# rajan-dubey8/camouflage-multimodal

Measured on AMD Instinct MI355X. Metric: images/sec fwd+bwd (fusion model train step: fwd + loss + bwd + clip + AdamW), higher is better.
Workload: dtype bf16; 1 GPU; BASELINE configs[1] on the path that exists (SURVEY 8d): cross-attention fusion model, packed variable-Nr minibatch (Nr ~ real 303..530 histogram, mean 483), Nk=13 real KG rows, train mode dropout 0.3, random-init weights; batch_per_gpu=16, global_batch=16, rg_dim=128, hidden_dim=256, num_heads=8, parallelism=dp1, precision=bf16 MFMA operands, fp32 accumulate/optimizer

## Files before the change

camouflage_multimodal_amd/csrc/common.h:

```cpp
#pragma once
#include <hip/hip_runtime.h>
#include <stdint.h>

#define CAMO_WAVE 64

enum : uint32_t {
  SITE_ATTN_RG2KG = 1, SITE_ATTN_KG2RG = 2, SITE_FFN_RG = 3, SITE_FFN_KG = 4, SITE_FUSE = 5,
  SITE_HEAD0 = 6,
  SITE_LATE0 = 10
};
enum : uint32_t { SITE_RGT_CONV0 = 32 , SITE_RGT_SHARED = 36, SITE_RGT_HEADS = 37 };

struct DropCfg {
  uint32_t seed_lo, seed_hi;
  float p;
  float scale;
  uint32_t thr;
};

__host__ __device__ inline DropCfg make_drop(int training, float p, uint64_t seed) {
  DropCfg d;
  d.seed_lo = (uint32_t)(seed & 0xFFFFFFFFull);
  d.seed_hi = (uint32_t)(seed >> 32);
  d.p = (training && p > 0.f) ? p : 0.f;
  d.scale = d.p > 0.f ? 1.0f / (1.0f - d.p) : 1.0f;
  const double t = (double)d.p * 16777216.0;
  unsigned long long t24 = (unsigned long long)t;
  if ((double)t24 < t) ++t24;
  d.thr = t24 >= 16777216ull ? 0xFFFFFFFFu : (uint32_t)(t24 << 8);
  return d;
}

__device__ __forceinline__ uint32_t fmix32(uint32_t x) {
  x ^= x >> 16; x *= 0x85EBCA6Bu; x ^= x >> 13; x *= 0xC2B2AE35u; x ^= x >> 16;
  return x;
}

__device__ __forceinline__ float drop_mult(const DropCfg& d, uint32_t site, uint32_t idx) {
  const uint32_t x = fmix32((idx + (site * 0x85EBCA77u + d.seed_lo)) ^ d.seed_hi);
  return x >= d.thr ? d.scale : 0.0f;
}

extern "C" __device__ int camo_writelane_i32(int, int, int) __asm("llvm.amdgcn.writelane.i32");
#define SET_LANE(v, s, i) (v) = (uint32_t)camo_writelane_i32((int)(s), (i), (int)(v))

__device__ __forceinline__ float wave_sum(float v) {
#pragma unroll
  for (int o = 32; o > 0; o >>= 1) v += __shfl_xor(v, o, 64);
  return v;
}
template <int CTRL, int ROWMASK>
__device__ __forceinline__ float dpp_add(float v) {
  return v + __int_as_float(__builtin_amdgcn_update_dpp(0, __float_as_int(v), CTRL, ROWMASK, 0xf, true));
}
__device__ __forceinline__ float wave_sum_lane63(float v) {
  v = dpp_add<0x111, 0xf>(v);
  v = dpp_add<0x112, 0xf>(v);
  v = dpp_add<0x114, 0xf>(v);
  v = dpp_add<0x118, 0xf>(v);
  v = dpp_add<0x142, 0xa>(v);
  v = dpp_add<0x143, 0xc>(v);
  return v;
}
__device__ __forceinline__ float wave_max(float v) {
// ... 65 lines not shown
```

camouflage_multimodal_amd/csrc/fused_rows.hip:

```cpp
#include "fused_rows.h"
#include "shadow_inl.h"
#include "gemm.h"
#include "mfma_inl.h"

namespace {

template <int NT, int KS, bool W_IS_A, int DEPTH, bool USE_ROT = true>
struct Stage {
  static constexpr int TOTAL = NT * KS;
  static constexpr int D = DEPTH < TOTAL ? DEPTH : TOTAL;
  static_assert(!USE_ROT || (KS & (KS - 1)) == 0, "rotated k order: power-of-two k steps");
  u32x4 buf[D];
  const u32x4* wp; int rot;
  __device__ __forceinline__ int keff(int ks) const { return USE_ROT ? ((ks + rot) & (KS - 1)) : ks; }
  __device__ __forceinline__ const u32x4* wptr(int i) const { return wp + 64 * (keff(i / NT) * NT + (i % NT)); }
  __device__ __forceinline__ void prefetch(const u32x4* __restrict__ wp_, int rot_) {
    wp = wp_; rot = rot_;
#pragma unroll
    for (int i = 0; i < D; ++i) buf[i] = *wptr(i);
  }
  __device__ __forceinline__ void run(const char* act, f32x16 (&acc)[NT]) {
    run_f([&](int ks) { return *reinterpret_cast<const bf16x8*>(act + 32 * ks); }, acc);
  }
  template <class F>
  __device__ __forceinline__ void run_f(F&& frag, f32x16 (&acc)[NT]) {
    bf16x8 x = frag(keff(0)), xn = x;
#pragma unroll
    for (int i = 0; i < TOTAL; ++i) {
      const int ks = i / NT, t = i % NT;
      const bf16x8 wf = as_frag(buf[i % D]);
      if (i + D < TOTAL) buf[i % D] = *wptr(i + D);
      if (t == 0) {
        x = xn;
        if (ks + 1 < KS) xn = frag(keff(ks + 1));
      }
      if constexpr (W_IS_A) acc[t] = __builtin_amdgcn_mfma_f32_32x32x16_bf16(wf, x, acc[t], 0, 0, 0);
      else                  acc[t] = __builtin_amdgcn_mfma_f32_32x32x16_bf16(x, wf, acc[t], 0, 0, 0);
      __builtin_amdgcn_sched_barrier(0);
    }
  }
};

__device__ __forceinline__ void stamp(unsigned long long* stamps, int k) {
  if (stamps && threadIdx.x == 0) stamps[(size_t)blockIdx.x * 8 + k] = __builtin_amdgcn_s_memrealtime();
}

template <int LOG2C>
__device__ __forceinline__ void copy_out(const char* lds, int pitch, int col_byte0, us16* dst, int ld, size_t row0, int nrows) {
  for (int c = threadIdx.x; c < (32 << LOG2C); c += 256) {
    const int r = c >> LOG2C, k = c & ((1 << LOG2C) - 1);
    if (r < nrows)
      store16_wt(reinterpret_cast<char*>(dst + (row0 + r) * (size_t)ld) + 16 * k, *reinterpret_cast<const u32x4*>(lds + r * pitch + col_byte0 + 16 * k));
  }
}

__global__ __launch_bounds__(256) void shadow_kernel(const ShadowBatch sb, int total_chunks) {
  const int gid = blockIdx.x * 256 + threadIdx.x;
  for (int zi = 0; zi < sb.nzero; ++zi) {
    u32x4* z = static_cast<u32x4*>(sb.zero_ptr[zi]);
    const size_t n16 = sb.zero_bytes[zi] >> 4;
    for (size_t i = gid; i < n16; i += (size_t)gridDim.x * 256) z[i] = u32x4{0u, 0u, 0u, 0u};
  }
  if (gid >= total_chunks) return;
  int ji = 0;
#pragma unroll
  for (int i = 1; i < SHADOW_MAXJ; ++i)
    if (i < sb.n && gid >= sb.j[i].chunk_begin) ji = i;
// ... 7 lines not shown
  extern __shared__ __attribute__((aligned(16))) char smem[];
  const FrontStream& S = a.s[(int)blockIdx.x >= a.s[1].tile_begin ? 1 : 0];
  const int tid = threadIdx.x, lane = tid & 63, l31 = lane & 31, h = lane >> 5;
  const int w = __builtin_amdgcn_readfirstlane(tid >> 6);
  const int row0 = ((int)blockIdx.x - S.tile_begin) * 32;
  const int nrows = min(32, S.M - row0);
  char* bufX = smem; char* bufR = smem + F_BUFR; char* bufQ = smem + F_BUFQ;
  const int rot = ROT ? (int)(blockIdx.x >> 3) : 0;
  stamp(a.stamps, 0);
  Stage<2, 8, true, DEPTH> st0;
  st0.prefetch(reinterpret_cast<const u32x4*>(S.W0) + (size_t)w * (8 * 2 * 64) + lane, rot);
  float* ptab = reinterpret_cast<float*>(smem + F_PTAB);
  {
    const int r = tid >> 3, c = tid & 7;
    const float4* src = reinterpret_cast<const float4*>(S.X + (size_t)(row0 + min(r, nrows - 1)) * 128 + 16 * c);
    float4 v0 = src[0], v1 = src[1], v2 = src[2], v3 = src[3];
    const float p0 = S.b0[tid], p1 = S.bq[tid], p2 = S.bkv[tid], p3 = S.bkv[256 + tid];
    ptab[tid] = p0; ptab[256 + tid] = p1; ptab[512 + tid] = p2; ptab[768 + tid] = p3;
    if (r >= nrows) { v0 = v1 = v2 = v3 = make_float4(0.f, 0.f, 0.f, 0.f); }
    *reinterpret_cast<u32x4*>(bufX + r * PX + 32 * c) = u32x4{pack2(v0.x, v0.y), pack2(v0.z, v0.w), pack2(v1.x, v1.y), pack2(v1.z, v1.w)};
    *reinterpret_cast<u32x4*>(bufX + r * PX + 32 * c + 16) = u32x4{pack2(v2.x, v2.y), pack2(v2.z, v2.w), pack2(v3.x, v3.y), pack2(v3.z, v3.w)};
  }
  __syncthreads();
  Stage<6, 16, true, DEPTH> st1;
  {
    f32x16 acc[2] = {zero16(), zero16()};
    st0.run(bufX + l31 * PX + 16 * h, acc);
    st1.prefetch(reinterpret_cast<const u32x4*>(S.W1) + (size_t)w * (16 * 6 * 64) + lane, rot);
#pragma unroll
    for (int t = 0; t < 2; ++t)
#pragma unroll
      for (int g = 0; g < 4; ++g) {
        const int c0 = 64 * w + 32 * t + 8 * g + 4 * h;
        const float4 bv = *reinterpret_cast<const float4*>(ptab + c0);
        *reinterpret_cast<u32x2*>(bufR + l31 * PR + 2 * c0) =
            u32x2{pack2(acc[t][4 * g] + bv.x, acc[t][4 * g + 1] + bv.y), pack2(acc[t][4 * g + 2] + bv.z, acc[t][4 * g + 3] + bv.w)};
      }
  }
  __syncthreads();
  stamp(a.stamps, 1);
  {
    f32x16 acc[6];
#pragma unroll
    for (int t = 0; t < 6; ++t) acc[t] = zero16();
    st1.run(bufR + l31 * PR + 16 * h, acc);
#pragma unroll
    for (int t = 0; t < 6; ++t) {
      const int tg = 6 * w + t;
      const float* bias = ptab + 256 + 32 * tg;
      const float sc = tg < 8 ? a.qscale : 1.0f;
#pragma unroll
      for (int g = 0; g < 4; ++g) {
        const int c = 8 * g + 4 * h;
        const float4 bv = *reinterpret_cast<const float4*>(bias + c);
        *reinterpret_cast<u32x2*>(bufQ + l31 * PQ + 2 * (32 * tg + c)) =
            u32x2{pack2((acc[t][4 * g] + bv.x) * sc, (acc[t][4 * g + 1] + bv.y) * sc),
                  pack2((acc[t][4 * g + 2] + bv.z) * sc, (acc[t][4 * g + 3] + bv.w) * sc)};
      }
    }
  }
  __syncthreads();
  stamp(a.stamps, 2);
  copy_out<5>(bufQ, PQ, 0, S.Q16, 256, row0, nrows);
  copy_out<6>(bufQ, PQ, 512, S.KV16, 512, row0, nrows);
  copy_out<5>(bufR, PR, 0, S.R16, 256, row0, nrows);
  if (a.save) copy_out<4>(bufX, PX, 0, S.X16, 128, row0, nrows);
  for (int zi = 0; zi < a.nzero; ++zi) {
    u32x4* z = static_cast<u32x4*>(a.zero_ptr[zi]);
    const unsigned n16 = a.zero_bytes[zi] >> 4;
    for (unsigned i = blockIdx.x * 256 + tid; i < n16; i += gridDim.x * 256) z[i] = u32x4{0u, 0u, 0u, 0u};
  }
  stamp(a.stamps, 3);
}

constexpr int PK = 528;
constexpr int PVC = 192;
constexpr int PT = 260;
constexpr int B_VS = 16 * PK;
template <int OCC> struct BackL;
template <> struct BackL<2> { static constexpr int XH = 0, O = 32 * PT * 4, Y = O + 32 * PR, RED = Y + 32 * PR, PTAB = RED + 1024, LDS = PTAB + 5120; };
template <> struct BackL<3> { static constexpr int Y = 0, XH = 32 * PR, O = 2 * 32 * PR, RED = O + 32 * PR, LDS = RED + 1024; };
constexpr int B_LDS = BackL<2>::LDS;
// ... 62 lines not shown
  const us16* kbase = a.KV2_16 + (size_t)rb * 512 + 64 * w + 8 * h;
  const us16* vbase = a.KV2_16 + (size_t)rb * 512 + 256 + 64 * w;
  bf16x8 qf[2][2];
  u32x4 kf[2][2][2], vv[2][4];
#pragma unroll
  for (int hd = 0; hd < 2; ++hd)
#pragma unroll
    for (int s = 0; s < 2; ++s) qf[hd][s] = as_frag(*reinterpret_cast<const u32x4*>(qrow + 32 * hd + 16 * s));
#pragma unroll
  for (int c = 0; c < 2; ++c) {
    const us16* p = kbase + (size_t)min(r0 + 32 * c + l31, nr - 1) * 512;
#pragma unroll
    for (int hd = 0; hd < 2; ++hd)
#pragma unroll
      for (int s = 0; s < 2; ++s) kf[c][hd][s] = *reinterpret_cast<const u32x4*>(p + 32 * hd + 16 * s);
  }
#pragma unroll
  for (int c = 0; c < 2; ++c)
#pragma unroll
    for (int i = 0; i < 4; ++i) {
      const int id = lane + 64 * i;
      vv[c][i] = *reinterpret_cast<const u32x4*>(vbase + (size_t)min(r0 + 32 * c + (id >> 3), nr - 1) * 512 + 8 * (id & 7));
    }
  f32x16 S[2][2];
  float mx[2] = {-INFINITY, -INFINITY};
#pragma unroll
  for (int c = 0; c < 2; ++c)
#pragma unroll
    for (int hd = 0; hd < 2; ++hd) {
      S[c][hd] = zero16();
#pragma unroll
      for (int s = 0; s < 2; ++s) S[c][hd] = __builtin_amdgcn_mfma_f32_32x32x16_bf16(as_frag(kf[c][hd][s]), qf[hd][s], S[c][hd], 0, 0, 0);
#pragma unroll
      for (int i = 0; i < 16; ++i) mx[hd] = (r0 + 32 * c + acc_row(i, h) < nr) ? fmaxf(mx[hd], S[c][hd][i]) : mx[hd];
    }
  mx[0] = fmaxf(mx[0], __shfl_xor(mx[0], 32, 64));
  mx[1] = fmaxf(mx[1], __shfl_xor(mx[1], 32, 64));
  stamp(a.stamps, 1);
  f32x16 Z[2] = {zero16(), zero16()};
  float L[2] = {0.f, 0.f};
  const bool dodrop = a.drop.p > 0.f;
  const int q4 = (lane >> 2) & 3, p4 = lane & 3, g1 = (lane >> 4) & 1;
#pragma unroll
  for (int c = 0; c < 2; ++c) {
#pragma unroll
    for (int i = 0; i < 4; ++i) { const int id = lane + 64 * i; *reinterpret_cast<u32x4*>(Vt + (id >> 3) * PVC + 16 * (id & 7)) = vv[c][i]; }
#pragma unroll
    for (int hd = 0; hd < 2; ++hd) {
      float e[16];
#pragma unroll
      for (int i = 0; i < 16; ++i) {
        const int row = r0 + 32 * c + acc_row(i, h);
        e[i] = row < nr ? __expf(S[c][hd][i] - mx[hd]) : 0.f;
        L[hd] += e[i];
        if (dodrop) e[i] *= drop_mult(a.drop, SITE_ATTN_KG2RG, ((uint32_t)(rb + row) * 8u + (uint32_t)(2 * w + hd)) * (uint32_t)Nk + (uint32_t)l31);
      }
#pragma unroll
      for (int s = 0; s < 2; ++s) {
        const bf16x8 ef = as_frag(u32x4{pack2(e[8 * s], e[8 * s + 1]), pack2(e[8 * s + 2], e[8 * s + 3]),
                                        pack2(e[8 * s + 4], e[8 * s + 5]), pack2(e[8 * s + 6], e[8 * s + 7])});
        const char* vp = Vt + (16 * s + 4 * h + q4) * PVC + 2 * (32 * hd + 16 * g1 + 4 * p4);
        const bf16x8 vf = join(lds_tr16(vp), lds_tr16(vp + 8 * PVC));
        Z[hd] = __builtin_amdgcn_mfma_f32_32x32x16_bf16(ef, vf, Z[hd], 0, 0, 0);
      }
    }
  }
  L[0] += __shfl_xor(L[0], 32, 64);
  L[1] += __shfl_xor(L[1], 32, 64);
  stamp(a.stamps, 2);
#pragma unroll
  for (int hd = 0; hd < 2; ++hd) {
    float* part = a.part + (((size_t)a.tile_off[b] + 2 * sp) * 8 + 2 * w + hd) * PART_FLOATS;
    if (lane < 16) {
      __hip_atomic_store(part + lane, mx[hd], __ATOMIC_RELAXED, __HIP_MEMORY_SCOPE_AGENT);
      __hip_atomic_store(part + 16 + lane, L[hd], __ATOMIC_RELAXED, __HIP_MEMORY_SCOPE_AGENT);
    }
    float* zt = reinterpret_cast<float*>(Vt);
#pragma unroll
// ... 81 lines not shown
      *reinterpret_cast<u32x2*>(bufO + j * PR + 2 * (32 * hd + 4 * f4)) =
          u32x2{pack2(acc[it][0] * il, acc[it][1] * il), pack2(acc[it][2] * il, acc[it][3] * il)};
    }
  }
}

template <int DEPTH, bool ROT, int OCC>
__global__ __launch_bounds__(256, OCC) void back_kernel(const BackArgs a) {
  extern __shared__ __attribute__((aligned(16))) char smem[];
  const int tid = threadIdx.x, lane = tid & 63, l31 = lane & 31, h = lane >> 5;
  const int w = __builtin_amdgcn_readfirstlane(tid >> 6);
  const int nkg = a.B * a.max_splits;
  const int vid = (int)blockIdx.x < a.lead_tiles ? nkg + (int)blockIdx.x : ((int)blockIdx.x < a.lead_tiles + nkg ? (int)blockIdx.x - a.lead_tiles : (int)blockIdx.x);
  const bool kg = vid < nkg;
  int rot = ROT ? (int)(blockIdx.x >> 3) : 0;
  using L = BackL<OCC>;
  char* bufO = smem + L::O; char* bufY = smem + L::Y;
  float* red = reinterpret_cast<float*>(smem + L::RED);
  float* tile32 = reinterpret_cast<float*>(smem);
  int b; size_t rowg0; int nrows; float inv_n;
  stamp(a.stamps, 0);
  const BackStream& S = a.s[kg ? 1 : 0];
  Stage<2, 16, true, DEPTH> sto;
  Stage<4, 16, false, DEPTH> stf;
  if (!kg) sto.prefetch(reinterpret_cast<const u32x4*>(S.Wo) + (size_t)w * (16 * 2 * 64) + lane, rot);
  float* ptab = reinterpret_cast<float*>(smem + BackL<2>::PTAB);
  float pt[5];
  u32x2 rres[2][4];
  auto load_early = [&](size_t row) {
    if constexpr (OCC == 2) {
      pt[0] = S.bo[tid]; pt[1] = S.ln_g[tid]; pt[2] = S.ln_b[tid]; pt[3] = S.b1[tid]; pt[4] = S.b1[256 + tid];
#pragma unroll
      for (int t = 0; t < 2; ++t)
#pragma unroll
        for (int g = 0; g < 4; ++g) rres[t][g] = *reinterpret_cast<const u32x2*>(S.R16 + row * 256 + 64 * w + 32 * t + 8 * g + 4 * h);
    }
  };
  if (kg) {
    b = vid / a.max_splits;
    const int sp = vid - b * a.max_splits;
    if (ROT) rot = b;
    const int nsplit = (a.off[b + 1] - a.off[b] + SPLIT_ROWS - 1) / SPLIT_ROWS;
    if (sp >= nsplit) return;
    attn_kg_split(a, smem, b, sp, w, lane);
    stamp(a.stamps, 4);
    asm volatile("s_waitcnt vmcnt(0)" ::: "memory");
    __syncthreads();
// ... 17 lines not shown
    const int4 td = a.tile_desc[vid - nkg];
    if (td.x < 0) return;
    b = td.x; rowg0 = td.y; nrows = td.z; inv_n = __int_as_float(td.w);
    load_early(rowg0 + min(l31, nrows - 1));
    attn_rg_tile(a, smem, bufO, b, rowg0, nrows, w, lane);
  }
  if constexpr (OCC == 2) {
#pragma unroll
    for (int i = 0; i < 5; ++i) ptab[256 * i + tid] = pt[i];
  }
  __syncthreads();
  stamp(a.stamps, 1);
  auto pvec = [&](const float* g, int at, int c) {
    if constexpr (OCC == 2) return *reinterpret_cast<const float4*>(ptab + at + c);
    else return *reinterpret_cast<const float4*>(g + c);
  };

  const size_t rrow = rowg0 + min(l31, nrows - 1);
  float u[32];
  float rstd_keep = 0.f;
  {
    f32x16 acc[2] = {zero16(), zero16()};
    sto.run(bufO + l31 * PR + 16 * h, acc);
    stf.prefetch(reinterpret_cast<const u32x4*>(S.W1) + (size_t)w * (16 * 4 * 64) + lane, rot);
    float part = 0.f;
#pragma unroll
    for (int t = 0; t < 2; ++t)
#pragma unroll
      for (int g = 0; g < 4; ++g) {
        const int c0 = 64 * w + 32 * t + 8 * g + 4 * h;
        const float4 bv = pvec(S.bo, 0, c0);
        u32x2 rv;
        if constexpr (OCC == 2) rv = rres[t][g];
        else rv = *reinterpret_cast<const u32x2*>(S.R16 + rrow * 256 + c0);
        float* o = u + 16 * t + 4 * g;
        o[0] = acc[t][4 * g] + bv.x + bf_lo(rv.x); o[1] = acc[t][4 * g + 1] + bv.y + bf_hi(rv.x);
        o[2] = acc[t][4 * g + 2] + bv.z + bf_lo(rv.y); o[3] = acc[t][4 * g + 3] + bv.w + bf_hi(rv.y);
        part += (o[0] + o[1]) + (o[2] + o[3]);
      }
    auto row_total = [&](float p, int slot) {
      p += __shfl_xor(p, 32, 64);
      if (h == 0) red[slot * 128 + w * 32 + l31] = p;
      __syncthreads();
      return (red[slot * 128 + l31] + red[slot * 128 + 32 + l31]) + (red[slot * 128 + 64 + l31] + red[slot * 128 + 96 + l31]);
    };
    const float mean = row_total(part, 0) * (1.0f / 256.0f);
    float sq = 0.f;
// ... 31 lines not shown
          const float send = up ? ys[i] : ys[i + n];
          const float keep = up ? ys[i + n] : ys[i];
          ys[i] = keep + __shfl_xor(send, m, 64);
        }
      }
      const float tot = ys[0] + __shfl_xor(ys[0], 1, 64);
      if ((l31 & 1) == 0) {
        const int i16 = (l31 >> 1) & 15;
        atomicAdd(S.Ymean + (size_t)b * 256 + 64 * w + 32 * t + 8 * (i16 >> 2) + 4 * h + (i16 & 3), tot * inv_n);
      }
    }
  }
  __syncthreads();
  stamp(a.stamps, 2);
  float ymean_keep = 0.f;
  if constexpr (OCC == 2) {
    float sum = 0.f;
    for (int r = 0; r < nrows; ++r) sum += tile32[r * PT + tid];
    ymean_keep = sum * inv_n;
  }

  {
    f32x16 acc[4] = {zero16(), zero16(), zero16(), zero16()};
    stf.run(bufY + l31 * PR + 16 * h, acc);
    if constexpr (OCC == 2) atomicAdd(S.Ymean + (size_t)b * 256 + tid, ymean_keep);
    const bool dodrop = a.drop.p > 0.f;
#pragma unroll
    for (int t = 0; t < 4; ++t) {
      const int f = 128 * w + 32 * t + l31;
      float bias;
      if constexpr (OCC == 2) bias = ptab[768 + f];
      else bias = S.b1[f];
      float colsum = 0.f;
      uint32_t wlo = 0u, whi = 0u;
#pragma unroll
      for (int i = 0; i < 16; ++i) {
        if (8 * (i >> 2) >= nrows) continue;
        const int row = acc_row(i, h);
        float v = fmaxf(acc[t][i] + bias, 0.f);
        if (dodrop) v *= drop_mult(a.drop, S.site_ffn, (uint32_t)(rowg0 + row) * 512u + (uint32_t)f);
        if (row >= nrows) v = 0.f;
        colsum += v;
        if (a.save) {
          const unsigned long long bal = __ballot(v > 0.f);
          SET_LANE(wlo, (uint32_t)bal, i); SET_LANE(whi, (uint32_t)(bal >> 32), i);
        }
      }
      colsum += __shfl_xor(colsum, 32, 64);
      if (h == 0) atomicAdd(S.Hmean + (size_t)b * 512 + f, colsum * inv_n);
      if (a.save && lane < 16) {
        const int ra = acc_row(lane, 0);
        if (ra < nrows) S.mask[(rowg0 + ra) * 16 + 4 * w + t] = wlo;
        if (ra + 4 < nrows) S.mask[(rowg0 + ra + 4) * 16 + 4 * w + t] = whi;
      }
    }
  }
  if (a.save) {
    char* bufXH = smem + L::XH;
    if (w == 0 && h == 0 && l31 < nrows) S.rstd[rowg0 + l31] = rstd_keep;
    __syncthreads();
    if constexpr (OCC == 2) {
#pragma unroll
      for (int t = 0; t < 2; ++t)
#pragma unroll
        for (int g = 0; g < 4; ++g) {
          const float* o = u + 16 * t + 4 * g;
          *reinterpret_cast<u32x2*>(bufXH + l31 * PR + 2 * (64 * w + 32 * t + 8 * g + 4 * h)) = u32x2{pack2(o[0], o[1]), pack2(o[2], o[3])};
        }
      __syncthreads();
    }
    copy_out<5>(bufXH, PR, 0, S.XH16, 256, rowg0, nrows);
    copy_out<5>(bufO, PR, 0, S.O16, 256, rowg0, nrows);
    copy_out<5>(bufY, PR, 0, S.Y16, 256, rowg0, nrows);
  }
  stamp(a.stamps, 3);
}
// ... 117 lines not shown
  const bool rok = l31 < nrows;
  float* ptab = reinterpret_cast<float*>(smem + W_PTAB);
  const float rstd = S.rstd[vrow];
  const float ptv0 = S.dcomb[(size_t)b * S.ld_dcomb + tid], ptv1 = S.ln_g[tid];
  u32x2 xv[2][4], ov[2][4];
#pragma unroll
  for (int t = 0; t < 2; ++t)
#pragma unroll
    for (int g = 0; g < 4; ++g) {
      const int c0 = 64 * w + 32 * t + 8 * g + 4 * h;
      xv[t][g] = *reinterpret_cast<const u32x2*>(S.XH16 + vrow * 256 + c0);
    }
  if (kg) {
#pragma unroll
    for (int t = 0; t < 2; ++t)
#pragma unroll
      for (int g = 0; g < 4; ++g) ov[t][g] = *reinterpret_cast<const u32x2*>(a.O2_16 + vrow * 256 + 64 * w + 32 * t + 8 * g + 4 * h);
  }
  const float dh0 = S.dHm[(size_t)b * S.ld_dHm + tid], dh1 = S.dHm[(size_t)b * S.ld_dHm + 256 + tid];
  u32x4 mw[4];
#pragma unroll
  for (int i = 0; i < 4; ++i) mw[i] = reinterpret_cast<const u32x4*>(S.mask + vrow * 16)[i];
  u32x4 qreg[4];
  if (!kg) {
#pragma unroll
    for (int i = 0; i < 4; ++i) {
      const int id = tid + 256 * i;
      qreg[i] = *reinterpret_cast<const u32x4*>(a.Q16 + (rowg0 + min(id >> 5, nrows - 1)) * 256 + 8 * (id & 31));
    }
    u32x4 kv[4];
#pragma unroll
    for (int i = 0; i < 4; ++i) {
      const int c = tid + 256 * i;
      kv[i] = *reinterpret_cast<const u32x4*>(a.KV16 + ((size_t)b * a.Nk + min(c >> 6, a.Nk - 1)) * 512 + 8 * (c & 63));
    }
#pragma unroll
    for (int i = 0; i < 4; ++i) {
      const int c = tid + 256 * i, j = c >> 6, ch = c & 63;
      const u32x4 v = j < a.Nk ? kv[i] : u32x4{0u, 0u, 0u, 0u};
      if (ch < 32) *reinterpret_cast<u32x4*>(Ks + j * PK + 16 * ch) = v;
      else         *reinterpret_cast<u32x4*>(Vs + j * PK + 16 * (ch - 32)) = v;
    }
  }
  {
    const float gs = inv_n * a.drop.scale;
    gtab[tid] = f2bf(dh0 * gs); gtab[256 + tid] = f2bf(dh1 * gs);
  }
  ptab[tid] = ptv0; ptab[256 + tid] = ptv1;
#pragma unroll
  for (int t = 0; t < 2; ++t)
#pragma unroll
    for (int g = 0; g < 4; ++g) {
      const int c0 = 64 * w + 32 * t + 8 * g + 4 * h;
      *reinterpret_cast<u32x2*>(bufdU + l31 * PR + 2 * c0) = xv[t][g];
      if (kg) *reinterpret_cast<u32x2*>(Ks + l31 * PR + 2 * c0) = ov[t][g];
    }
  __syncthreads();
// ... 86 lines not shown
        dot = fmaf(acc2[t][4 * g], bf_lo(ov.x), dot); dot = fmaf(acc2[t][4 * g + 1], bf_hi(ov.x), dot);
        dot = fmaf(acc2[t][4 * g + 2], bf_lo(ov.y), dot); dot = fmaf(acc2[t][4 * g + 3], bf_hi(ov.y), dot);
        if (rok) *reinterpret_cast<u32x2*>(a.dO2_16 + (rowg0 + l31) * 256 + c0) =
            u32x2{pack2(acc2[t][4 * g], acc2[t][4 * g + 1]), pack2(acc2[t][4 * g + 2], acc2[t][4 * g + 3])};
      }
      dot += __shfl_xor(dot, 32, 64);
      if (h == 0 && rok) a.delta2[((size_t)b * 8 + 2 * w + t) * 16 + l31] = dot;
    }
    stamp(a.stamps, 3);
    return;
  }
  __syncthreads();
#pragma unroll
  for (int i = 0; i < 4; ++i) { const int id = tid + 256 * i; *reinterpret_cast<u32x4*>(bufQ + (id >> 5) * PR + 16 * (id & 31)) = qreg[i]; }
#pragma unroll
  for (int t = 0; t < 2; ++t)
#pragma unroll
    for (int g = 0; g < 4; ++g) {
      const int c0 = 64 * w + 32 * t + 8 * g + 4 * h;
      *reinterpret_cast<u32x2*>(bufdO + l31 * PR + 2 * c0) =
          rok ? u32x2{pack2(acc2[t][4 * g], acc2[t][4 * g + 1]), pack2(acc2[t][4 * g + 2], acc2[t][4 * g + 3])} : u32x2{0u, 0u};
    }
  __syncthreads();
  const bool dodrop = a.drop.p > 0.f;
  const int q4 = (lane >> 2) & 3, p4 = lane & 3, g1 = (lane >> 4) & 1;
#pragma unroll
  for (int t = 0; t < 2; ++t) {
    const int head = 2 * w + t;
    f32x16 Sc = zero16();
#pragma unroll
    for (int s = 0; s < 2; ++s) {
      const bf16x8 kf = *reinterpret_cast<const bf16x8*>(Ks + (l31 & 15) * PK + 2 * (32 * head + 16 * s + 8 * h));
      const bf16x8 qf = *reinterpret_cast<const bf16x8*>(bufQ + l31 * PR + 2 * (32 * head + 16 * s + 8 * h));
      Sc = __builtin_amdgcn_mfma_f32_32x32x16_bf16(kf, qf, Sc, 0, 0, 0);
    }
    float pr[8], mm[8];
    rg_softmax(Sc, h, a.Nk, pr);
    const uint32_t ibase = ((uint32_t)(rowg0 + l31) * 8u + (uint32_t)head) * (uint32_t)a.Nk;
#pragma unroll
    for (int i = 0; i < 8; ++i) mm[i] = dodrop ? drop_mult(a.drop, SITE_ATTN_RG2KG, ibase + (uint32_t)acc_row(i, h)) : 1.0f;
    f32x16 dP = zero16();
#pragma unroll
    for (int s = 0; s < 2; ++s) {
      const char* vp = Vs + (l31 & 15) * PK + 2 * (32 * head + 16 * s + 4 * h);
      const u32x2 v0 = *reinterpret_cast<const u32x2*>(vp), v1 = *reinterpret_cast<const u32x2*>(vp + 16);
      const bf16x8 vf = as_frag(u32x4{v0.x, v0.y, v1.x, v1.y});
      const bf16x8 of = as_frag(u32x4{pack2(acc2[t][8 * s], acc2[t][8 * s + 1]), pack2(acc2[t][8 * s + 2], acc2[t][8 * s + 3]),
                                      pack2(acc2[t][8 * s + 4], acc2[t][8 * s + 5]), pack2(acc2[t][8 * s + 6], acc2[t][8 * s + 7])});
      dP = __builtin_amdgcn_mfma_f32_32x32x16_bf16(vf, of, dP, 0, 0, 0);
    }
    float ds[8], pd[8], delta = 0.f;
#pragma unroll
    for (int i = 0; i < 8; ++i) { ds[i] = dP[i] * mm[i]; delta = fmaf(pr[i], ds[i], delta); pd[i] = pr[i] * mm[i]; }
    delta += __shfl_xor(delta, 32, 64);
#pragma unroll
    for (int i = 0; i < 8; ++i) { ds[i] = rok ? pr[i] * (ds[i] - delta) : 0.f; if (!rok) pd[i] = 0.f; }
    const u32x4 dsf = u32x4{pack2(ds[0], ds[1]), pack2(ds[2], ds[3]), pack2(ds[4], ds[5]), pack2(ds[6], ds[7])};
    const u32x4 pdf = u32x4{pack2(pd[0], pd[1]), pack2(pd[2], pd[3]), pack2(pd[4], pd[5]), pack2(pd[6], pd[7])};
    {
      const char* kp = Ks + (4 * h + q4) * PK + 2 * (32 * head + 16 * g1 + 4 * p4);
      const bf16x8 kt = join(lds_tr16(kp), lds_tr16(kp + 8 * PK));
      const f32x16 dq = __builtin_amdgcn_mfma_f32_32x32x16_bf16(kt, as_frag(dsf), zero16(), 0, 0, 0);
      if (rok) {
// ... 206 lines not shown
#pragma unroll
  for (int i = 0; i < 4; ++i) {
    const int id = tid + 256 * i;
    const size_t r = rowg0 + min(id >> 5, nrows - 1);
    *reinterpret_cast<u32x4*>(bufT + (id >> 5) * PQ + 16 * (id & 31)) = *reinterpret_cast<const u32x4*>(a.KV2_16 + r * 512 + 8 * (id & 31));
    dqreg[i] = *reinterpret_cast<const u32x4*>(a.dQKV16 + r * 768 + 8 * (id & 31));
  }
  u32x2 dureg[2][4];
#pragma unroll
  for (int t = 0; t < 2; ++t)
#pragma unroll
    for (int g = 0; g < 4; ++g) dureg[t][g] = *reinterpret_cast<const u32x2*>(a.dU16 + vrow * 256 + 64 * w + 32 * t + 8 * g + 4 * h);
  bf16x8 kf[2][2], vf[2][2];
  {
    const us16* kp = a.KV2_16 + vrow * 512 + 64 * w + 8 * h;
#pragma unroll
    for (int t = 0; t < 2; ++t)
#pragma unroll
      for (int s = 0; s < 2; ++s) {
        kf[t][s] = as_frag(*reinterpret_cast<const u32x4*>(kp + 32 * t + 16 * s));
        vf[t][s] = as_frag(*reinterpret_cast<const u32x4*>(kp + 256 + 32 * t + 16 * s));
      }
  }
  __syncthreads();
  const bool dodrop = a.drop.p > 0.f;
  const int q4 = (lane >> 2) & 3, p4 = lane & 3, g1 = (lane >> 4) & 1;
#pragma unroll
  for (int t = 0; t < 2; ++t) {
    const int head = 2 * w + t;
    f32x16 S2 = zero16(), dP = zero16();
#pragma unroll
    for (int s = 0; s < 2; ++s) {
      const int co = (l31 & 15) * PK + 2 * (32 * head + 16 * s + 8 * h);
      S2 = __builtin_amdgcn_mfma_f32_32x32x16_bf16(*reinterpret_cast<const bf16x8*>(Q2s + co), kf[t][s], S2, 0, 0, 0);
      dP = __builtin_amdgcn_mfma_f32_32x32x16_bf16(*reinterpret_cast<const bf16x8*>(dO2s + co), vf[t][s], dP, 0, 0, 0);
    }
    float ds[8], pd[8];
#pragma unroll
    for (int i = 0; i < 8; ++i) {
      const int j = acc_row(i, h);
      const float p = (j < Nk && rok) ? __expf(S2[i] - tabs[head * 16 + j]) * tabs[128 + head * 16 + j] : 0.f;
      const float mm = dodrop ? drop_mult(a.drop, SITE_ATTN_KG2RG, ((uint32_t)(rowg0 + l31) * 8u + (uint32_t)head) * (uint32_t)Nk + (uint32_t)j) : 1.0f;
      ds[i] = p * (dP[i] * mm - tabs[256 + head * 16 + j]);
      pd[i] = p * mm;
    }
    const u32x4 dsf = u32x4{pack2(ds[0], ds[1]), pack2(ds[2], ds[3]), pack2(ds[4], ds[5]), pack2(ds[6], ds[7])};
    const u32x4 pdf = u32x4{pack2(pd[0], pd[1]), pack2(pd[2], pd[3]), pack2(pd[4], pd[5]), pack2(pd[6], pd[7])};
    const int tro = (4 * h + q4) * PK + 2 * (32 * head + 16 * g1 + 4 * p4);
    const f32x16 dv = __builtin_amdgcn_mfma_f32_32x32x16_bf16(join(lds_tr16(dO2s + tro), lds_tr16(dO2s + tro + 8 * PK)), as_frag(pdf), zero16(), 0, 0, 0);
    const f32x16 dk = __builtin_amdgcn_mfma_f32_32x32x16_bf16(join(lds_tr16(Q2s + tro), lds_tr16(Q2s + tro + 8 * PK)), as_frag(dsf), zero16(), 0, 0, 0);
#pragma unroll
    for (int g = 0; g < 4; ++g) {
      const int c = 32 * head + 8 * g + 4 * h;
      *reinterpret_cast<u32x2*>(bufT + l31 * PQ + 2 * (256 + c)) = u32x2{pack2(dk[4 * g], dk[4 * g + 1]), pack2(dk[4 * g + 2], dk[4 * g + 3])};
      *reinterpret_cast<u32x2*>(bufT + l31 * PQ + 2 * (512 + c)) = u32x2{pack2(dv[4 * g], dv[4 * g + 1]), pack2(dv[4 * g + 2], dv[4 * g + 3])};
    }
    char* im = imgs + head * 1024;
    *reinterpret_cast<u32x2*>(im + l31 * 32 + 8 * h) = u32x2{dsf.x, dsf.y};
    *reinterpret_cast<u32x2*>(im + l31 * 32 + 16 + 8 * h) = u32x2{dsf.z, dsf.w};
    f32x16 dq2 = zero16();
#pragma unroll
    for (int s = 0; s < 2; ++s) {
      const int r0 = 16 * s + 8 * h + q4;
      const bf16x8 sA = join(lds_tr16(im + r0 * 32 + 8 * p4), lds_tr16(im + (r0 + 4) * 32 + 8 * p4));
      const int co = 2 * (32 * head + 16 * g1 + 4 * p4);
// ... 133 lines not shown
    const size_t o = (size_t)b * 128 + tid;
    const bool ok = j < Nk;
    tabs[tid] = ok ? a.lse2[2 * o] : 0.f;
    tabs[128 + tid] = ok ? 1.0f / a.lse2[2 * o + 1] : 0.f;
    tabs[256 + tid] = ok ? a.delta2[o] : 0.f;
  }
#pragma unroll
  for (int i = 0; i < 4; ++i) {
    const int id = tid + 256 * i;
    const size_t r = rowg0 + min(id >> 5, nrows - 1);
    *reinterpret_cast<u32x4*>(bufT + (id >> 5) * PQ + 16 * (id & 31)) = *reinterpret_cast<const u32x4*>(a.KV2_16 + r * 512 + 8 * (id & 31));
  }
  bf16x8 kf[2][2], vf[2][2];
  {
    const us16* kp = a.KV2_16 + vrow * 512 + 64 * w + 8 * h;
#pragma unroll
    for (int t = 0; t < 2; ++t)
#pragma unroll
      for (int s = 0; s < 2; ++s) {
        kf[t][s] = as_frag(*reinterpret_cast<const u32x4*>(kp + 32 * t + 16 * s));
        vf[t][s] = as_frag(*reinterpret_cast<const u32x4*>(kp + 256 + 32 * t + 16 * s));
      }
  }
  __syncthreads();
  const bool dodrop = a.drop.p > 0.f;
  const int q4 = (lane >> 2) & 3, p4 = lane & 3, g1 = (lane >> 4) & 1;
#pragma unroll
  for (int t = 0; t < 2; ++t) {
    const int head = 2 * w + t;
    f32x16 S2 = zero16(), dP = zero16();
#pragma unroll
    for (int s = 0; s < 2; ++s) {
      const int co = (l31 & 15) * PK + 2 * (32 * head + 16 * s + 8 * h);
      S2 = __builtin_amdgcn_mfma_f32_32x32x16_bf16(*reinterpret_cast<const bf16x8*>(Q2s + co), kf[t][s], S2, 0, 0, 0);
      dP = __builtin_amdgcn_mfma_f32_32x32x16_bf16(*reinterpret_cast<const bf16x8*>(dO2s + co), vf[t][s], dP, 0, 0, 0);
    }
    float ds[8], pd[8];
#pragma unroll
    for (int i = 0; i < 8; ++i) {
      const int j = acc_row(i, h);
      const float p = (j < Nk && rok) ? __expf(S2[i] - tabs[head * 16 + j]) * tabs[128 + head * 16 + j] : 0.f;
      const float mm = dodrop ? drop_mult(a.drop, SITE_ATTN_KG2RG, ((uint32_t)(rowg0 + l31) * 8u + (uint32_t)head) * (uint32_t)Nk + (uint32_t)j) : 1.0f;
      ds[i] = p * (dP[i] * mm - tabs[256 + head * 16 + j]);
      pd[i] = p * mm;
    }
    const u32x4 dsf = u32x4{pack2(ds[0], ds[1]), pack2(ds[2], ds[3]), pack2(ds[4], ds[5]), pack2(ds[6], ds[7])};
    const u32x4 pdf = u32x4{pack2(pd[0], pd[1]), pack2(pd[2], pd[3]), pack2(pd[4], pd[5]), pack2(pd[6], pd[7])};
    const int tro = (4 * h + q4) * PK + 2 * (32 * head + 16 * g1 + 4 * p4);
    const f32x16 dv = __builtin_amdgcn_mfma_f32_32x32x16_bf16(join(lds_tr16(dO2s + tro), lds_tr16(dO2s + tro + 8 * PK)), as_frag(pdf), zero16(), 0, 0, 0);
    const f32x16 dk = __builtin_amdgcn_mfma_f32_32x32x16_bf16(join(lds_tr16(Q2s + tro), lds_tr16(Q2s + tro + 8 * PK)), as_frag(dsf), zero16(), 0, 0, 0);
#pragma unroll
    for (int g = 0; g < 4; ++g) {
      const int c = 32 * head + 8 * g + 4 * h;
      *reinterpret_cast<u32x2*>(bufT + l31 * PQ + 2 * (256 + c)) = u32x2{pack2(dk[4 * g], dk[4 * g + 1]), pack2(dk[4 * g + 2], dk[4 * g + 3])};
      *reinterpret_cast<u32x2*>(bufT + l31 * PQ + 2 * (512 + c)) = u32x2{pack2(dv[4 * g], dv[4 * g + 1]), pack2(dv[4 * g + 2], dv[4 * g + 3])};
    }
    char* im = imgs + head * 1024;
    *reinterpret_cast<u32x2*>(im + l31 * 32 + 8 * h) = u32x2{dsf.x, dsf.y};
    *reinterpret_cast<u32x2*>(im + l31 * 32 + 16 + 8 * h) = u32x2{dsf.z, dsf.w};
    f32x16 dq2 = zero16();
#pragma unroll
    for (int s = 0; s < 2; ++s) {
      const int r0 = 16 * s + 8 * h + q4;
      const bf16x8 sA = join(lds_tr16(im + r0 * 32 + 8 * p4), lds_tr16(im + (r0 + 4) * 32 + 8 * p4));
      const int co = 2 * (32 * head + 16 * g1 + 4 * p4);
// ... 196 lines not shown
```

Measured before the change: 104,300 images/s.

## Interleave GEMM epilogues into MFMA loop and precompute dropout keep masks

Adds a tile-major Stage order whose loop takes a side callback, so each finished output tile's bias/scale/ReLU/dropout epilogue runs under the next tile's MFMAs instead of after the whole GEMM. Dropout hashes for the attention kernels are now computed into bitmasks early, overlapping the load and barrier latency, and the hot loops just test a bit. The aim is to hide epilogue VALU work and hash cost behind matrix-core and memory work. The trade-off is more live registers (extra accumulators, bias and colsum arrays), which may hurt occupancy or cause spills.

```diff
diff --git a/camouflage_multimodal_amd/csrc/common.h b/camouflage_multimodal_amd/csrc/common.h
--- a/camouflage_multimodal_amd/csrc/common.h
+++ b/camouflage_multimodal_amd/csrc/common.h
@@ -36,10 +36,14 @@
   return x;
 }
 
+__device__ __forceinline__ bool drop_keep(const DropCfg& d, uint32_t site, uint32_t idx) {
+  const uint32_t x = fmix32((idx + (site * 0x85EBCA77u + d.seed_lo)) ^ d.seed_hi);
+  return x >= d.thr;
+}
 __device__ __forceinline__ float drop_mult(const DropCfg& d, uint32_t site, uint32_t idx) {
-  const uint32_t x = fmix32((idx + (site * 0x85EBCA77u + d.seed_lo)) ^ d.seed_hi);
-  return x >= d.thr ? d.scale : 0.0f;
+  return drop_keep(d, site, idx) ? d.scale : 0.0f;
 }
+__device__ __forceinline__ float keep_mult(const DropCfg& d, uint32_t bits, int k) { return (bits >> k) & 1u ? d.scale : 0.0f; }
 
 extern "C" __device__ int camo_writelane_i32(int, int, int) __asm("llvm.amdgcn.writelane.i32");
 #define SET_LANE(v, s, i) (v) = (uint32_t)camo_writelane_i32((int)(s), (i), (int)(v))
diff --git a/camouflage_multimodal_amd/csrc/fused_rows.hip b/camouflage_multimodal_amd/csrc/fused_rows.hip
--- a/camouflage_multimodal_amd/csrc/fused_rows.hip
+++ b/camouflage_multimodal_amd/csrc/fused_rows.hip
@@ -5,44 +5,67 @@
 
 namespace {
 
-template <int NT, int KS, bool W_IS_A, int DEPTH, bool USE_ROT = true>
+template <int NT, int KS, bool W_IS_A, int DEPTH, bool USE_ROT = true, bool TILE_MAJOR = false>
 struct Stage {
   static constexpr int TOTAL = NT * KS;
   static constexpr int D = DEPTH < TOTAL ? DEPTH : TOTAL;
+  static constexpr int XSTEP = TILE_MAJOR ? 1 : NT;
   static_assert(!USE_ROT || (KS & (KS - 1)) == 0, "rotated k order: power-of-two k steps");
   u32x4 buf[D];
-  const u32x4* wp; int rot;
+  const u32x4* wp; int rot; unsigned ln = 0u;
+  static __device__ __forceinline__ constexpr int step_ks(int i) { return TILE_MAJOR ? i % KS : i / NT; }
+  static __device__ __forceinline__ constexpr int step_t(int i) { return TILE_MAJOR ? i / KS : i % NT; }
   __device__ __forceinline__ int keff(int ks) const { return USE_ROT ? ((ks + rot) & (KS - 1)) : ks; }
-  __device__ __forceinline__ const u32x4* wptr(int i) const { return wp + 64 * (keff(i / NT) * NT + (i % NT)); }
+  __device__ __forceinline__ const u32x4* wptr(int i) const {
+    if constexpr (TILE_MAJOR) {
+      const char* kbase = reinterpret_cast<const char*>(wp) + (size_t)(keff(step_ks(i)) * (NT * 1024));
+      return reinterpret_cast<const u32x4*>(kbase + (size_t)(uint32_t)(16u * ln + 1024u * (unsigned)step_t(i)));
+    } else {
+      return wp + 64 * (keff(step_ks(i)) * NT + step_t(i)) + ln;
+    }
+  }
   __device__ __forceinline__ void prefetch(const u32x4* __restrict__ wp_, int rot_) {
     wp = wp_; rot = rot_;
 #pragma unroll
     for (int i = 0; i < D; ++i) buf[i] = *wptr(i);
   }
+  __device__ __forceinline__ void prefetch(const u32x4* __restrict__ wave_stream, int lane, int rot_) {
+    ln = (unsigned)lane;
+    prefetch(wave_stream, rot_);
+  }
   __device__ __forceinline__ void run(const char* act, f32x16 (&acc)[NT]) {
-    run_f([&](int ks) { return *reinterpret_cast<const bf16x8*>(act + 32 * ks); }, acc);
+    run_fs([&](int ks) { return *reinterpret_cast<const bf16x8*>(act + 32 * ks); }, acc, [](int) {});
+  }
+  template <class S>
+  __device__ __forceinline__ void run_s(const char* act, f32x16 (&acc)[NT], S&& side) {
+    run_fs([&](int ks) { return *reinterpret_cast<const bf16x8*>(act + 32 * ks); }, acc, side);
   }
   template <class F>
-  __device__ __forceinline__ void run_f(F&& frag, f32x16 (&acc)[NT]) {
+  __device__ __forceinline__ void run_f(F&& frag, f32x16 (&acc)[NT]) { run_fs(frag, acc, [](int) {}); }
+  template <class F, class S>
+  __device__ __forceinline__ void run_fs(F&& frag, f32x16 (&acc)[NT], S&& side) {
     bf16x8 x = frag(keff(0)), xn = x;
 #pragma unroll
     for (int i = 0; i < TOTAL; ++i) {
-      const int ks = i / NT, t = i % NT;
+      const int t = step_t(i);
       const bf16x8 wf = as_frag(buf[i % D]);
       if (i + D < TOTAL) buf[i % D] = *wptr(i + D);
-      if (t == 0) {
+      if (i % XSTEP == 0) {
         x = xn;
-        if (ks + 1 < KS) xn = frag(keff(ks + 1));
-      }
-      if constexpr (W_IS_A) acc[t] = __builtin_amdgcn_mfma_f32_32x32x16_bf16(wf, x, acc[t], 0, 0, 0);
-      else                  acc[t] = __builtin_amdgcn_mfma_f32_32x32x16_bf16(x, wf, acc[t], 0, 0, 0);
+        if (i + XSTEP < TOTAL) xn = frag(keff(step_ks(i + XSTEP)));
+      }
+      const f32x16 c = (TILE_MAJOR && step_ks(i) == 0) ? zero16() : acc[t];
+      if constexpr (W_IS_A) acc[t] = __builtin_amdgcn_mfma_f32_32x32x16_bf16(wf, x, c, 0, 0, 0);
+      else                  acc[t] = __builtin_amdgcn_mfma_f32_32x32x16_bf16(x, wf, c, 0, 0, 0);
+      side(i);
       __builtin_amdgcn_sched_barrier(0);
     }
   }
 };
 
 __device__ __forceinline__ void stamp(unsigned long long* stamps, int k) {
-  if (stamps && threadIdx.x == 0) stamps[(size_t)blockIdx.x * 8 + k] = __builtin_amdgcn_s_memrealtime();
+  typedef __attribute__((address_space(1))) unsigned long long global_u64;
+  if (stamps && threadIdx.x == 0) ((global_u64*)stamps)[(size_t)blockIdx.x * 8 + k] = __builtin_amdgcn_s_memrealtime();
 }
 
 template <int LOG2C>
@@ -96,11 +119,11 @@
     *reinterpret_cast<u32x4*>(bufX + r * PX + 32 * c + 16) = u32x4{pack2(v2.x, v2.y), pack2(v2.z, v2.w), pack2(v3.x, v3.y), pack2(v3.z, v3.w)};
   }
   __syncthreads();
-  Stage<6, 16, true, DEPTH> st1;
+  Stage<6, 16, true, DEPTH, true, true> st1;
   {
     f32x16 acc[2] = {zero16(), zero16()};
     st0.run(bufX + l31 * PX + 16 * h, acc);
-    st1.prefetch(reinterpret_cast<const u32x4*>(S.W1) + (size_t)w * (16 * 6 * 64) + lane, rot);
+    st1.prefetch(reinterpret_cast<const u32x4*>(S.W1) + (size_t)w * (16 * 6 * 64), lane, rot);
 #pragma unroll
     for (int t = 0; t < 2; ++t)
 #pragma unroll
@@ -117,21 +140,22 @@
     f32x16 acc[6];
 #pragma unroll
     for (int t = 0; t < 6; ++t) acc[t] = zero16();
-    st1.run(bufR + l31 * PR + 16 * h, acc);
-#pragma unroll
-    for (int t = 0; t < 6; ++t) {
+    auto epi = [&](int t, int g) {
       const int tg = 6 * w + t;
       const float* bias = ptab + 256 + 32 * tg;
       const float sc = tg < 8 ? a.qscale : 1.0f;
-#pragma unroll
-      for (int g = 0; g < 4; ++g) {
-        const int c = 8 * g + 4 * h;
-        const float4 bv = *reinterpret_cast<const float4*>(bias + c);
-        *reinterpret_cast<u32x2*>(bufQ + l31 * PQ + 2 * (32 * tg + c)) =
-            u32x2{pack2((acc[t][4 * g] + bv.x) * sc, (acc[t][4 * g + 1] + bv.y) * sc),
-                  pack2((acc[t][4 * g + 2] + bv.z) * sc, (acc[t][4 * g + 3] + bv.w) * sc)};
-      }
-    }
+      const int c = 8 * g + 4 * h;
+      const float4 bv = *reinterpret_cast<const float4*>(bias + c);
+      *reinterpret_cast<u32x2*>(bufQ + l31 * PQ + 2 * (32 * tg + c)) =
+          u32x2{pack2((acc[t][4 * g] + bv.x) * sc, (acc[t][4 * g + 1] + bv.y) * sc),
+                pack2((acc[t][4 * g + 2] + bv.z) * sc, (acc[t][4 * g + 3] + bv.w) * sc)};
+    };
+    st1.run_s(bufR + l31 * PR + 16 * h, acc, [&](int i) {
+      const int t = i >> 4, r = i & 15;
+      if (t > 0 && (r & 3) == 2) epi(t - 1, r >> 2);
+    });
+#pragma unroll
+    for (int g = 0; g < 4; ++g) epi(5, g);
   }
   __syncthreads();
   stamp(a.stamps, 2);
@@ -240,6 +264,20 @@
       const int id = lane + 64 * i;
       vv[c][i] = *reinterpret_cast<const u32x4*>(vbase + (size_t)min(r0 + 32 * c + (id >> 3), nr - 1) * 512 + 8 * (id & 7));
     }
+  const bool dodrop = a.drop.p > 0.f;
+  uint32_t keep[2] = {0u, 0u};
+  if (dodrop) {
+#pragma unroll
+    for (int c = 0; c < 2; ++c)
+#pragma unroll
+      for (int hd = 0; hd < 2; ++hd)
+#pragma unroll
+        for (int i = 0; i < 16; ++i) {
+          const int row = r0 + 32 * c + acc_row(i, h);
+          keep[c] |= (uint32_t)drop_keep(a.drop, SITE_ATTN_KG2RG, ((uint32_t)(rb + row) * 8u + (uint32_t)(2 * w + hd)) * (uint32_t)Nk + (uint32_t)l31) << (16 * hd + i);
+        }
+    __builtin_amdgcn_sched_barrier(0);
+  }
   f32x16 S[2][2];
   float mx[2] = {-INFINITY, -INFINITY};
 #pragma unroll
@@ -257,7 +295,6 @@
   stamp(a.stamps, 1);
   f32x16 Z[2] = {zero16(), zero16()};
   float L[2] = {0.f, 0.f};
-  const bool dodrop = a.drop.p > 0.f;
   const int q4 = (lane >> 2) & 3, p4 = lane & 3, g1 = (lane >> 4) & 1;
 #pragma unroll
   for (int c = 0; c < 2; ++c) {
@@ -271,7 +308,7 @@
         const int row = r0 + 32 * c + acc_row(i, h);
         e[i] = row < nr ? __expf(S[c][hd][i] - mx[hd]) : 0.f;
         L[hd] += e[i];
-        if (dodrop) e[i] *= drop_mult(a.drop, SITE_ATTN_KG2RG, ((uint32_t)(rb + row) * 8u + (uint32_t)(2 * w + hd)) * (uint32_t)Nk + (uint32_t)l31);
+        if (dodrop) e[i] *= keep_mult(a.drop, keep[c], 16 * hd + i);
       }
 #pragma unroll
       for (int s = 0; s < 2; ++s) {
@@ -399,7 +436,7 @@
   stamp(a.stamps, 0);
   const BackStream& S = a.s[kg ? 1 : 0];
   Stage<2, 16, true, DEPTH> sto;
-  Stage<4, 16, false, DEPTH> stf;
+  Stage<4, 16, false, DEPTH, true, true> stf;
   if (!kg) sto.prefetch(reinterpret_cast<const u32x4*>(S.Wo) + (size_t)w * (16 * 2 * 64) + lane, rot);
   float* ptab = reinterpret_cast<float*>(smem + BackL<2>::PTAB);
   float pt[5];
@@ -463,7 +500,7 @@
   {
     f32x16 acc[2] = {zero16(), zero16()};
     sto.run(bufO + l31 * PR + 16 * h, acc);
-    stf.prefetch(reinterpret_cast<const u32x4*>(S.W1) + (size_t)w * (16 * 4 * 64) + lane, rot);
+    stf.prefetch(reinterpret_cast<const u32x4*>(S.W1) + (size_t)w * (16 * 4 * 64), lane, rot);
     float part = 0.f;
 #pragma unroll
     for (int t = 0; t < 2; ++t)
@@ -541,36 +578,42 @@
 
   {
     f32x16 acc[4] = {zero16(), zero16(), zero16(), zero16()};
-    stf.run(bufY + l31 * PR + 16 * h, acc);
+    const bool dodrop = a.drop.p > 0.f;
+    float bias[4], colsum[4] = {0.f, 0.f, 0.f, 0.f};
+    uint32_t wlo[4] = {0u, 0u, 0u, 0u}, whi[4] = {0u, 0u, 0u, 0u};
+    auto epi = [&](int t, int i) {
+      if (8 * (i >> 2) >= nrows) return;
+      const int row = acc_row(i, h);
+      float v = fmaxf(acc[t][i] + bias[t], 0.f);
+      if (dodrop) v *= drop_mult(a.drop, S.site_ffn, (uint32_t)(rowg0 + row) * 512u + (uint32_t)(128 * w + 32 * t + l31));
+      if (row >= nrows) v = 0.f;
+      colsum[t] += v;
+      if (a.save) {
+        const unsigned long long bal = __ballot(v > 0.f);
+        SET_LANE(wlo[t], (uint32_t)bal, i); SET_LANE(whi[t], (uint32_t)(bal >> 32), i);
+      }
+    };
+    stf.run_s(bufY + l31 * PR + 16 * h, acc, [&](int i) {
+      const int t = i >> 4, r = i & 15;
+      if (r == 8) {
+        if constexpr (OCC == 2) bias[t] = ptab[768 + 128 * w + 32 * t + l31];
+        else bias[t] = S.b1[128 * w + 32 * t + l31];
+      }
+      if (t > 0) epi(t - 1, r);
+    });
+    stamp(a.stamps, 7);
     if constexpr (OCC == 2) atomicAdd(S.Ymean + (size_t)b * 256 + tid, ymean_keep);
-    const bool dodrop = a.drop.p > 0.f;
+#pragma unroll
+    for (int i = 0; i < 16; ++i) epi(3, i);
 #pragma unroll
     for (int t = 0; t < 4; ++t) {
       const int f = 128 * w + 32 * t + l31;
-      float bias;
-      if constexpr (OCC == 2) bias = ptab[768 + f];
-      else bias = S.b1[f];
-      float colsum = 0.f;
-      uint32_t wlo = 0u, whi = 0u;
-#pragma unroll
-      for (int i = 0; i < 16; ++i) {
-        if (8 * (i >> 2) >= nrows) continue;
-        const int row = acc_row(i, h);
-        float v = fmaxf(acc[t][i] + bias, 0.f);
-        if (dodrop) v *= drop_mult(a.drop, S.site_ffn, (uint32_t)(rowg0 + row) * 512u + (uint32_t)f);
-        if (row >= nrows) v = 0.f;
-        colsum += v;
-        if (a.save) {
-          const unsigned long long bal = __ballot(v > 0.f);
-          SET_LANE(wlo, (uint32_t)bal, i); SET_LANE(whi, (uint32_t)(bal >> 32), i);
-        }
-      }
-      colsum += __shfl_xor(colsum, 32, 64);
-      if (h == 0) atomicAdd(S.Hmean + (size_t)b * 512 + f, colsum * inv_n);
+      const float cs = colsum[t] + __shfl_xor(colsum[t], 32, 64);
+      if (h == 0) atomicAdd(S.Hmean + (size_t)b * 512 + f, cs * inv_n);
       if (a.save && lane < 16) {
         const int ra = acc_row(lane, 0);
-        if (ra < nrows) S.mask[(rowg0 + ra) * 16 + 4 * w + t] = wlo;
-        if (ra + 4 < nrows) S.mask[(rowg0 + ra + 4) * 16 + 4 * w + t] = whi;
+        if (ra < nrows) S.mask[(rowg0 + ra) * 16 + 4 * w + t] = wlo[t];
+        if (ra + 4 < nrows) S.mask[(rowg0 + ra + 4) * 16 + 4 * w + t] = whi[t];
       }
     }
   }
@@ -734,6 +777,8 @@
 #pragma unroll
   for (int i = 0; i < 4; ++i) mw[i] = reinterpret_cast<const u32x4*>(S.mask + vrow * 16)[i];
   u32x4 qreg[4];
+  const bool dodrop = a.drop.p > 0.f;
+  uint32_t keep = 0u;
   if (!kg) {
 #pragma unroll
     for (int i = 0; i < 4; ++i) {
@@ -745,6 +790,15 @@
     for (int i = 0; i < 4; ++i) {
       const int c = tid + 256 * i;
       kv[i] = *reinterpret_cast<const u32x4*>(a.KV16 + ((size_t)b * a.Nk + min(c >> 6, a.Nk - 1)) * 512 + 8 * (c & 63));
+    }
+    if (dodrop) {
+#pragma unroll
+      for (int t = 0; t < 2; ++t) {
+        const uint32_t ibase = ((uint32_t)(rowg0 + l31) * 8u + (uint32_t)(2 * w + t)) * (uint32_t)a.Nk;
+#pragma unroll
+        for (int i = 0; i < 8; ++i) keep |= (uint32_t)drop_keep(a.drop, SITE_ATTN_RG2KG, ibase + (uint32_t)acc_row(i, h)) << (8 * t + i);
+      }
+      __builtin_amdgcn_sched_barrier(0);
     }
 #pragma unroll
     for (int i = 0; i < 4; ++i) {
@@ -877,7 +931,6 @@
           rok ? u32x2{pack2(acc2[t][4 * g], acc2[t][4 * g + 1]), pack2(acc2[t][4 * g + 2], acc2[t][4 * g + 3])} : u32x2{0u, 0u};
     }
   __syncthreads();
-  const bool dodrop = a.drop.p > 0.f;
   const int q4 = (lane >> 2) & 3, p4 = lane & 3, g1 = (lane >> 4) & 1;
 #pragma unroll
   for (int t = 0; t < 2; ++t) {
@@ -891,9 +944,8 @@
     }
     float pr[8], mm[8];
     rg_softmax(Sc, h, a.Nk, pr);
-    const uint32_t ibase = ((uint32_t)(rowg0 + l31) * 8u + (uint32_t)head) * (uint32_t)a.Nk;
-#pragma unroll
-    for (int i = 0; i < 8; ++i) mm[i] = dodrop ? drop_mult(a.drop, SITE_ATTN_RG2KG, ibase + (uint32_t)acc_row(i, h)) : 1.0f;
+#pragma unroll
+    for (int i = 0; i < 8; ++i) mm[i] = dodrop ? keep_mult(a.drop, keep, 8 * t + i) : 1.0f;
     f32x16 dP = zero16();
 #pragma unroll
     for (int s = 0; s < 2; ++s) {
@@ -1146,8 +1198,18 @@
         vf[t][s] = as_frag(*reinterpret_cast<const u32x4*>(kp + 256 + 32 * t + 16 * s));
       }
   }
-  __syncthreads();
   const bool dodrop = a.drop.p > 0.f;
+  uint32_t keep = 0u;
+  if (dodrop) {
+#pragma unroll
+    for (int t = 0; t < 2; ++t) {
+      const uint32_t ibase = ((uint32_t)(rowg0 + l31) * 8u + (uint32_t)(2 * w + t)) * (uint32_t)Nk;
+#pragma unroll
+      for (int i = 0; i < 8; ++i) keep |= (uint32_t)drop_keep(a.drop, SITE_ATTN_KG2RG, ibase + (uint32_t)acc_row(i, h)) << (8 * t + i);
+    }
+    __builtin_amdgcn_sched_barrier(0);
+  }
+  __syncthreads();
   const int q4 = (lane >> 2) & 3, p4 = lane & 3, g1 = (lane >> 4) & 1;
 #pragma unroll
   for (int t = 0; t < 2; ++t) {
@@ -1164,7 +1226,7 @@
     for (int i = 0; i < 8; ++i) {
       const int j = acc_row(i, h);
       const float p = (j < Nk && rok) ? __expf(S2[i] - tabs[head * 16 + j]) * tabs[128 + head * 16 + j] : 0.f;
-      const float mm = dodrop ? drop_mult(a.drop, SITE_ATTN_KG2RG, ((uint32_t)(rowg0 + l31) * 8u + (uint32_t)head) * (uint32_t)Nk + (uint32_t)j) : 1.0f;
+      const float mm = dodrop ? keep_mult(a.drop, keep, 8 * t + i) : 1.0f;
       ds[i] = p * (dP[i] * mm - tabs[256 + head * 16 + j]);
       pd[i] = p * mm;
     }
@@ -1344,8 +1406,18 @@
         vf[t][s] = as_frag(*reinterpret_cast<const u32x4*>(kp + 256 + 32 * t + 16 * s));
       }
   }
-  __syncthreads();
   const bool dodrop = a.drop.p > 0.f;
+  uint32_t keep = 0u;
+  if (dodrop) {
+#pragma unroll
+    for (int t = 0; t < 2; ++t) {
+      const uint32_t ibase = ((uint32_t)(rowg0 + l31) * 8u + (uint32_t)(2 * w + t)) * (uint32_t)Nk;
+#pragma unroll
+      for (int i = 0; i < 8; ++i) keep |= (uint32_t)drop_keep(a.drop, SITE_ATTN_KG2RG, ibase + (uint32_t)acc_row(i, h)) << (8 * t + i);
+    }
+    __builtin_amdgcn_sched_barrier(0);
+  }
+  __syncthreads();
   const int q4 = (lane >> 2) & 3, p4 = lane & 3, g1 = (lane >> 4) & 1;
 #pragma unroll
   for (int t = 0; t < 2; ++t) {
@@ -1362,7 +1434,7 @@
     for (int i = 0; i < 8; ++i) {
       const int j = acc_row(i, h);
       const float p = (j < Nk && rok) ? __expf(S2[i] - tabs[head * 16 + j]) * tabs[128 + head * 16 + j] : 0.f;
-      const float mm = dodrop ? drop_mult(a.drop, SITE_ATTN_KG2RG, ((uint32_t)(rowg0 + l31) * 8u + (uint32_t)head) * (uint32_t)Nk + (uint32_t)j) : 1.0f;
+      const float mm = dodrop ? keep_mult(a.drop, keep, 8 * t + i) : 1.0f;
       ds[i] = p * (dP[i] * mm - tabs[256 + head * 16 + j]);
       pd[i] = p * mm;
     }
```

New measurement: 105,800 images/s, median of 6. 1.01x the previous value.
